# fperezgamonal/flownet2-tf

Measured on AMD Instinct MI355X. Metric: forward pairs/sec at 512x384 (FlowNet2), higher is better.
Workload: dtype f16x2 (split fp16 hi+lo operands, 3 fp16 MFMAs per product, fp32 accumulate); 1 GPU; FlowNet2 forward, batch=4 synthetic 512x384 pairs per GPU, seeded synthetic weights; pairs_per_gpu=4, parallelism=dp1 (no collective)

## Files before the change

flownet2-tf_amd/csrc/conv.hip:

```cpp
#include "conv_common.h"
#include <cstdlib>

namespace fn2 {

template <typename T, typename OutT, int TC, int WC, int WP>
__global__ void __launch_bounds__(256) conv_igemm_kernel(const ConvArgs p) {
  constexpr int CH = 16 / (int)sizeof(T);
  constexpr int BC = WC * TC * 16;
  constexpr int BP = WP * 64;
  constexpr int NT = 256;
  static_assert(WC * WP == 4, "4 waves per block");
  constexpr int NPR = BP / 64;
  constexpr int NWR = (BC * 4 + NT - 1) / NT;
  constexpr int WSWZ_BIT = (TC == 4) ? 5 : (TC == 2) ? 4 : 3;
  __shared__ uint4 lds[2][(BC + BP) * 4];

  const int tid = threadIdx.x, lane = tid & 63, wave = tid >> 6;
  const int wc = wave / WP, wp = wave % WP;
  const int cid = tid & 3;

  int pad_y = p.pad, pad_x = p.pad, oy_off = 0, ox_off = 0, osc = 1;
  const T* wgt = reinterpret_cast<const T*>(p.wgt);
  const int phase = blockIdx.z / p.splitk, split = blockIdx.z - phase * p.splitk;
  if (p.deconv) {
// ... 167 lines not shown
               p.out_c0;
#pragma unroll
    for (int t = 0; t < TC; ++t) {
      float v[4];
      const int co = cout_base + t * 4;
#pragma unroll
      for (int r = 0; r < 4; ++r) {
        float x = acc[t][pt][r] * p.out_scale + bias[t][r];
        if constexpr (sizeof(OutT) == 4) {
          if (p.accum && co + r < p.Cout) x += load_elem<OutT>(po + co + r);
          if (co + r < p.Cout) x = act_grad<OutT>(p, out, po + co + r, co + r, x);
        }
        if (p.act == FN2_ACT_LEAKY) x = leaky(x);
        v[r] = x;
      }
      if (p.vec_ok && co + 3 < p.Cout) {
        store4<OutT>(po + co, v[0], v[1], v[2], v[3]);
      } else {
#pragma unroll
        for (int r = 0; r < 4; ++r)
          if (co + r < p.Cout) store_elem<OutT>(po + co + r, v[r]);
      }
    }
  }
}

template <typename OutT>
__global__ void __launch_bounds__(256) splitk_finalize_kernel(const float* __restrict__ ws, const float* __restrict__ bias,
                                                              OutT* __restrict__ out, long npix, int ws_cs, int splitk,
                                                              int Cout, int out_cs, int out_c0, int act, int vec_ok,
                                                              float out_scale, int accum, const OutT* __restrict__ mask_y,
                                                              int mask_c0, int mask_c1, const float* __restrict__ up_src,
                                                              const float* __restrict__ up_w, const float* __restrict__ up_bias,
                                                              int up_c0, int out_H, int out_W) {
  const int groups = ws_cs / 4;
  const int groups_all = groups + (up_src != nullptr ? 1 : 0);
  const long total = npix * groups_all;
  const size_t slab = (size_t)npix * ws_cs;
  for (long i = (long)blockIdx.x * blockDim.x + threadIdx.x; i < total; i += (long)gridDim.x * blockDim.x) {
    const long pix = i / groups_all;
    const int co = (int)(i - pix * groups_all) * 4;
    if (co == groups * 4) {
      const int ox = (int)(pix % out_W), oy = (int)((pix / out_W) % out_H), n = (int)(pix / out_W / out_H);
      const int H = out_H >> 1, W = out_W >> 1;
      const int a = oy & 1, b = ox & 1, y = oy >> 1, x = ox >> 1;
      float r0 = up_bias ? up_bias[0] : 0.f, r1 = up_bias ? up_bias[1] : 0.f;
#pragma unroll
      for (int ty = 0; ty < 2; ++ty) {
        const int iy = y - 1 + a + ty, ky = 3 - a - 2 * ty;
        if (iy < 0 || iy >= H) continue;
#pragma unroll
        for (int tx = 0; tx < 2; ++tx) {
          const int ix = x - 1 + b + tx, kx = 3 - b - 2 * tx;
          if (ix < 0 || ix >= W) continue;
          const float2 v = *reinterpret_cast<const float2*>(up_src + (((long)n * H + iy) * W + ix) * 2);
          const float* ww = up_w + (ky * 4 + kx) * 4;
          r0 += v.x * ww[0] + v.y * ww[1];
          r1 += v.x * ww[2] + v.y * ww[3];
        }
      }
      OutT* pu = out + (size_t)pix * out_cs + up_c0;
      store_elem<OutT>(pu, r0);
      store_elem<OutT>(pu + 1, r1);
      continue;
    }
    float4 v = *reinterpret_cast<const float4*>(ws + pix * ws_cs + co);
    int s = 1;
    for (; s + 3 < splitk; s += 4) {
      float4 t[4];
#pragma unroll
      for (int u = 0; u < 4; ++u) t[u] = *reinterpret_cast<const float4*>(ws + (s + u) * slab + pix * ws_cs + co);
#pragma unroll
      for (int u = 0; u < 4; ++u) { v.x += t[u].x; v.y += t[u].y; v.z += t[u].z; v.w += t[u].w; }
    }
    for (; s < splitk; ++s) {
      const float4 t = *reinterpret_cast<const float4*>(ws + s * slab + pix * ws_cs + co);
      v.x += t.x; v.y += t.y; v.z += t.z; v.w += t.w;
    }
    float r[4] = {v.x, v.y, v.z, v.w};
    OutT* po = out + (size_t)pix * out_cs + out_c0 + co;
    const bool full = vec_ok && co + 3 < Cout;
    float old[4] = {0.f, 0.f, 0.f, 0.f}, yv[4] = {1.f, 1.f, 1.f, 1.f};
    const bool mask = mask_y != nullptr && co < mask_c1 && co + 4 > mask_c0;
    if constexpr (sizeof(OutT) == 4) {
      if (full) {
        if (accum) load4<OutT>(po, old);
        if (mask) load4<OutT>(mask_y + (size_t)pix * out_cs + out_c0 + co, yv);
      } else {
#pragma unroll
        for (int j = 0; j < 4; ++j)
          if (co + j < Cout) {
            if (accum) old[j] = load_elem<OutT>(po + j);
            if (mask) yv[j] = load_elem<OutT>(mask_y + (size_t)pix * out_cs + out_c0 + co + j);
          }
      }
    }
#pragma unroll
    for (int j = 0; j < 4; ++j) {
      r[j] *= out_scale;
      if (bias != nullptr && co + j < Cout) r[j] += bias[co + j];
// ... 697 lines not shown
  if (d->wgt_layout >= 1) {
    const long in_bytes = (long)d->in.n * d->in.h * d->in.w * d->in.cs * esz;
    FN2_REQUIRE(in_bytes < (1L << 31), "conv2d: input buffer >= 2 GiB is not addressable by the LDS-DMA kernel");
    FN2_REQUIRE((long)d->cout_pad * d->kpad * esz < (1L << 31), "conv2d: packed weight >= 2 GiB per phase");
    a.in_bytes = (int)in_bytes;
  }
  {
    const double A = (double)d->cout_pad * d->kpad * esz, B = (double)d->in.n * d->in.h * d->in.w * d->in.cs * esz;
    const long X = cdiv(M, 64), Y = cdiv(d->cout_pad, 128);
    const char* e = getenv("FN2_WMAJOR");
    const int mode = e ? atoi(e) : 2;
    a.wmajor = mode == 2 ? (A * (double)(X < 8 ? X : 8) + B > A + B * (double)(Y < 8 ? Y : 8)) : mode;
  }
  a.bp64 = wfrag ? 1 : wants_bp64(a, tile, phases, d->wgt_layout) ? 1 : 0;
  if ((a.dbg & 64) && d->wgt_layout == 1 && tile == 128 && !a.bp64) a.bp64 = 2;
  if (wfrag) {
    const char* e_wr = getenv("FN2_WREG_RING");
    const char* e_ring = getenv("FN2_RING_MAX");
    const int mode = e_wr ? atoi(e_wr) : 1;
    const long blocks = (long)cdiv(a.M, 64) * (a.cout_pad / 128) * phases;
    if (tile == 128 && (mode == 2 || (mode == 1 && blocks >= 384 && blocks <= (e_ring ? atoi(e_ring) : 512)))) a.wfrag = 2;
  }
  a.kg = 1;
  if (d->wgt_layout == 1 && tile == 128 && !(a.dbg & 32)) {
    const char* e_kg = getenv("FN2_KG");
    if (!e_kg || atoi(e_kg) != 0) {
      const char* e3 = getenv("FN2_KG3_MAX");
      const char* e2 = getenv("FN2_KG2_MAX");
      const long blocks = (long)cdiv(a.M, 64) * (a.cout_pad / 128) * phases;
      if (blocks <= (e3 ? atoi(e3) : 0)) { a.bp64 = 1; a.kg = 3; }
      else if (blocks <= (e2 ? atoi(e2) : 95)) { a.bp64 = 1; a.kg = 2; }
    }
  }
  if (d->wgt_layout == 1 && tile == 128 && !(a.dbg & 32) && d->in.dtype == FN2_F16X2) {
    const char* e_lo = getenv("FN2_DEEP_MIN");
    const char* e_hi = getenv("FN2_DEEP_MAX");
    const long blocks = (long)cdiv(a.M, 64) * (a.cout_pad / 128) * phases;
    const int lo = e_lo ? atoi(e_lo) : 0, hi = e_hi ? atoi(e_hi) : -1;
    if (blocks >= lo && blocks <= hi) { a.bp64 = 3; a.kg = 1; }
  }
  if (d->wgt_layout == 1 && tile == 128 && a.bp64 == 1 && a.kg == 1) {
    const char* e_ring = getenv("FN2_RING_MAX");
    const int ring_max = e_ring ? atoi(e_ring) : 512;
    const long blocks = (long)cdiv(a.M, 64) * (a.cout_pad / 128) * phases;
    if ((a.dbg & 256) || (blocks >= 384 && blocks <= ring_max)) a.bp64 = 2;
    const char* e_rs = getenv("FN2_RING_SPLIT");
    if (e_rs && blocks >= atoi(e_rs) && blocks < 384) a.bp64 = 2;
  }
  *tile_out = tile;
  *phases_out = phases;
  return FN2_OK;
}

static int preferred_split(const ConvArgs& a, int tile, int phases) {
  if (a.merged) return 1;
  const int bp = tile == 128 ? (a.bp64 ? 64 : 128) : (a.bp64 ? 128 : 256);
  const long blocks = (long)cdiv(a.M, bp) * (a.cout_pad / tile) * phases;
  const char* e_min = getenv("FN2_SPLIT_MINBLOCKS");
  if (blocks >= (e_min ? atoi(e_min) : 384)) return 1;
  if (a.bp64 == 3) {
    const char* e_sl = getenv("FN2_DEEP_SLOTS");
    int s = (int)((e_sl ? atoi(e_sl) : 256) / blocks);
    const int maxs = a.ksteps / 16;
    if (s > maxs) s = maxs;
    if (s > 16) s = 16;
    if (s < 2) return 1;
    const int kper = cdiv(a.ksteps, s);
    return cdiv(a.ksteps, kper);
  }
  if (a.kg > 1) {
    const char* e_nos = getenv("FN2_KG_NOSPLIT");
    if (blocks >= (e_nos ? atoi(e_nos) : 96)) return 1;
    const char* e_sl = getenv("FN2_KG_SLOTS");
    int s = (int)((e_sl ? atoi(e_sl) : 256) / blocks);
    const int maxs = a.ksteps / (12 * a.kg);
    if (s > maxs) s = maxs;
    if (s > 16) s = 16;
    if (s < 2) return 1;
    const int kper = cdiv(a.ksteps, s);
    return cdiv(a.ksteps, kper);
  }
  const char* e = getenv("FN2_SPLIT_SLOTS");
  const char* e_rsl = getenv("FN2_RING_SPLIT_SLOTS");
  const int slots = (tile == 128 && a.bp64 == 2) ? (e_rsl ? atoi(e_rsl) : 512) : e ? atoi(e) : 640;
  int s = (int)(slots / blocks);
  const int maxs = a.ksteps / 8;
  if (s > maxs) s = maxs;
  if (s > 16) s = 16;
  if (s < 2) return 1;
  const int kper = cdiv(a.ksteps, s);
  return cdiv(a.ksteps, kper);
}

static int64_t split_bytes(const ConvArgs& a, int s) {
  return (int64_t)s * a.N * a.out_H * a.out_W * a.ws_cs * (int64_t)sizeof(float);
}

}

extern "C" {

int64_t fn2_conv2d_workspace_bytes(const fn2_conv_desc* d) {
  ConvArgs a;
  int tile, phases;
  if (build_args(d, &a, &tile, &phases) != FN2_OK) return 0;
  if (is_flow_head(d)) return 0;
  const int s = preferred_split(a, tile, phases);
  return s > 1 ? split_bytes(a, s) : 0;
}

int fn2_conv2d_splits(const fn2_conv_desc* d) {
  ConvArgs a;
  int tile, phases;
  if (build_args(d, &a, &tile, &phases) != FN2_OK || is_flow_head(d)) return 1;
  int sk = preferred_split(a, tile, phases);
  while (sk > 1 && (d->workspace == nullptr || split_bytes(a, sk) > d->workspace_bytes)) --sk;
  if ((long)a.N * a.out_H * a.out_W * a.ws_cs >= (1L << 31)) sk = 1;
  if (sk > 1) {
    const int kper = cdiv(a.ksteps, sk);
    sk = cdiv(a.ksteps, kper);
    if (d->wgt_layout >= 1) sk = cdiv(a.ksteps / 2, cdiv(kper, 2));
  }
  return sk < 1 ? 1 : sk;
}

int fn2_conv2d_kernel_name(const fn2_conv_desc* d, char* name, int cap) {
  FN2_REQUIRE(name && cap > 0, "conv2d_kernel_name: no buffer");
  name[0] = 0;
  if (!d || d->wgt_layout < 1 || is_flow_head(d)) return FN2_OK;
  conv_name_sink() = ConvNameSink{name, cap};
  const int rc = fn2_conv2d(d, nullptr);
  conv_name_sink() = ConvNameSink{nullptr, 0};
  return rc;
}

int fn2_conv2d(const fn2_conv_desc* d, void* stream) {
  ConvArgs a;
  int tile, phases;
  int rc = build_args(d, &a, &tile, &phases);
  if (rc) return rc;
  hipStream_t s = (hipStream_t)stream;
  if (is_flow_head(d)) {
    int blocks = grid_for((long)a.M * 64, 256);
    if (d->in.dtype == FN2_F16X2 && a.M <= 4096 && !(a.dbg & 32768)) {
      a.dbg |= 16384;
      blocks = a.M;
    } else {
      a.dbg &= ~16384;
    }
    if (d->in.dtype == FN2_F32)
      hipLaunchKernelGGL(flow_head_kernel<float>, dim3(blocks), dim3(256), 0, s, a);
    else if (d->in.dtype == FN2_BF16)
      hipLaunchKernelGGL(flow_head_kernel<bf16_t>, dim3(blocks), dim3(256), 0, s, a);
    else if (d->in.dtype == FN2_F16)
      hipLaunchKernelGGL(flow_head_kernel<f16_t>, dim3(blocks), dim3(256), 0, s, a);
    else
      hipLaunchKernelGGL(flow_head_kernel<x2_t>, dim3(blocks), dim3(256), 0, s, a);
    FN2_CHECK_LAUNCH("flow_head");
    return FN2_OK;
  }
  int sk = preferred_split(a, tile, phases);
  while (sk > 1 && (d->workspace == nullptr || split_bytes(a, sk) > d->workspace_bytes)) --sk;
  if ((long)a.N * a.out_H * a.out_W * a.ws_cs >= (1L << 31)) sk = 1;
  if (sk > 1) {
    a.kper = cdiv(a.ksteps, sk);
    sk = cdiv(a.ksteps, a.kper);
  }
  if (sk > 1) {
    a.splitk = sk;
    a.ws = reinterpret_cast<float*>(d->workspace);
  }
  if (d->up_src != nullptr && d->kind == 5 && 2 * d->out.c == 32) {
    a.up_src = d->up_src; a.up_w = d->up_w; a.up_bias = d->up_bias; a.up_c0 = d->up_c0;
  }
  if (d->head != nullptr && !conv_name_sink().buf) {
    const fn2_conv_desc* h = reinterpret_cast<const fn2_conv_desc*>(d->head);
    FN2_REQUIRE(d->kind == 1 && is_flow_head(h) && h->head == nullptr && h->up_src == nullptr,
                "conv2d: head rides on a kind-1 transposed conv and is a 3x3 two-output fp32 flow head");
    FN2_REQUIRE(h->in.data == d->in.data && h->in.n == d->in.n && h->in.h == d->in.h && h->in.w == d->in.w &&
                    h->in.cs == d->in.cs && h->in.c0 == d->in.c0 && h->in.dtype == d->in.dtype,
                "conv2d: head and transposed conv must read the same view");
    ConvArgs ha;
    int htile, hphases;
    rc = build_args(h, &ha, &htile, &hphases);
    if (rc) return rc;
    const char* e = getenv("FN2_HEAD_RIDE");
    const bool ride = d->in.dtype == FN2_F16X2 && d->wgt_layout == 2 && tile == 128 && sk > 1 && !(e && atoi(e) == 0);
    if (ride) {
      a.fh_M = ha.M;
      a.fh_w = reinterpret_cast<const float*>(ha.wgt);
      a.fh_w1 = ha.ksteps * 4 * 4;
      a.fh_groups = ha.cin_chunks >> 1;
      a.fh_bias = ha.bias;
      a.fh_out = reinterpret_cast<float*>(ha.out);
      a.fh_out_cs = ha.out_cs; a.fh_out_c0 = ha.out_c0;
      a.fh_scale = ha.out_scale;
    } else {
      rc = fn2_conv2d(h, stream);
      if (rc) return rc;
    }
  }
  if (d->wgt_layout >= 1) {
    a.ksteps = a.ksteps / 2;
    a.kper = cdiv(a.kper, 2);
    a.splitk = cdiv(a.ksteps, a.kper);
    if (a.splitk == 1) a.ws = nullptr;
    rc = launch_conv_fast(a, d->in.dtype, d->out.dtype, tile, phases, s);
  } else if (d->in.dtype == FN2_F32 && d->out.dtype == FN2_F16X2) rc = launch_conv<float, x2_t>(a, tile, phases, s);
  else if (d->in.dtype == FN2_F32) rc = launch_conv<float, float>(a, tile, phases, s);
  else if (d->in.dtype == FN2_BF16 && d->out.dtype == FN2_BF16) rc = launch_conv<bf16_t, bf16_t>(a, tile, phases, s);
  else if (d->in.dtype == FN2_BF16) rc = launch_conv<bf16_t, float>(a, tile, phases, s);
  else if (d->out.dtype == FN2_F16) rc = launch_conv<f16_t, f16_t>(a, tile, phases, s);
  else rc = launch_conv<f16_t, float>(a, tile, phases, s);
  if (rc || conv_name_sink().buf) return rc;
  if (a.splitk == 1) {
    if (d->up_src == nullptr || a.up_src != nullptr) return rc;
    fn2_tensor uv = d->out;
    uv.c = 2; uv.c0 = d->up_c0;
    return fn2_upsample_flow(d->up_src, d->up_w, d->up_bias, &uv, d->out.n, d->out.h / 2, d->out.w / 2, stream);
  }
  if ((a.dbg & 524288) || d->raw_partials) return rc;
  const long npix = (long)a.N * a.out_H * a.out_W;
  const int fgrid = grid_for(npix * (a.ws_cs / 4 + (d->up_src != nullptr ? 1 : 0)), 256);
  if (d->out.dtype == FN2_F32)
    hipLaunchKernelGGL(splitk_finalize_kernel<float>, dim3(fgrid), dim3(256), 0, s, a.ws, a.bias, (float*)a.out, npix,
                       a.ws_cs, a.splitk, a.Cout, a.out_cs, a.out_c0, a.act, a.vec_ok, a.out_scale, a.accum, (const float*)a.mask_y, a.mask_c0, a.mask_c1, d->up_src, d->up_w, d->up_bias, d->up_c0, a.out_H, a.out_W);
  else if (d->out.dtype == FN2_F16X2)
    hipLaunchKernelGGL(splitk_finalize_kernel<x2_t>, dim3(fgrid), dim3(256), 0, s, a.ws, a.bias, (x2_t*)a.out,
                       npix, a.ws_cs, a.splitk, a.Cout, a.out_cs, a.out_c0, a.act, a.vec_ok, a.out_scale, a.accum, (const x2_t*)a.mask_y, a.mask_c0, a.mask_c1, d->up_src, d->up_w, d->up_bias, d->up_c0, a.out_H, a.out_W);
  else if (d->out.dtype == FN2_BF16)
    hipLaunchKernelGGL(splitk_finalize_kernel<bf16_t>, dim3(fgrid), dim3(256), 0, s, a.ws, a.bias, (bf16_t*)a.out,
                       npix, a.ws_cs, a.splitk, a.Cout, a.out_cs, a.out_c0, a.act, a.vec_ok, a.out_scale, a.accum, (const bf16_t*)a.mask_y, a.mask_c0, a.mask_c1, d->up_src, d->up_w, d->up_bias, d->up_c0, a.out_H, a.out_W);
  else
    hipLaunchKernelGGL(splitk_finalize_kernel<f16_t>, dim3(fgrid), dim3(256), 0, s, a.ws, a.bias, (f16_t*)a.out,
                       npix, a.ws_cs, a.splitk, a.Cout, a.out_cs, a.out_c0, a.act, a.vec_ok, a.out_scale, a.accum, (const f16_t*)a.mask_y, a.mask_c0, a.mask_c1, d->up_src, d->up_w, d->up_bias, d->up_c0, a.out_H, a.out_W);
  FN2_CHECK_LAUNCH("splitk_finalize");
  return FN2_OK;
}

int fn2_flow_head_gather(const float* t, int t_cs, const float* bias, float* out, int n, int h, int w, void* stream) {
  FN2_REQUIRE(t && out, "flow_head_gather: null pointer");
  FN2_REQUIRE(t_cs >= 18 && t_cs % 2 == 0 && n >= 1 && h >= 1 && w >= 1, "flow_head_gather: t must hold 18 partials per pixel");
  const long tiles = (long)n * ((h + GT_Y - 1) / GT_Y) * ((w + GT_X - 1) / GT_X);
  if (tiles >= 1024)
    hipLaunchKernelGGL(flow_head_gather_kernel, dim3((unsigned)std::min<long>(tiles, 1 << 16)), dim3(256), 0,
                       (hipStream_t)stream, t, t_cs, bias, out, n, h, w);
  else
    hipLaunchKernelGGL(flow_head_gather_small_kernel, dim3(grid_for((long)n * h * w, 256)), dim3(256), 0,
                       (hipStream_t)stream, t, t_cs, bias, out, n, h, w);
  FN2_CHECK_LAUNCH("flow_head_gather");
  return FN2_OK;
}

int fn2_flow_head_tail(const float* t, int t_cs, int taps, const float* bias, float* pf, int n, int h, int w, int ring,
                       const float* up_w, const float* up_bias, const fn2_tensor* up_out, void* stream) {
  return fn2_flow_head_tail_slabs(t, t_cs, 1, 0, 1.f, taps, bias, pf, n, h, w, ring, up_w, up_bias, up_out, stream);
}

int fn2_flow_head_tail_slabs(const float* t, int t_cs, int nslab, int64_t slab_stride, float scale, int taps, const float* bias,
                             float* pf, int n, int h, int w, int ring, const float* up_w, const float* up_bias,
                             const fn2_tensor* up_out, void* stream) {
  FN2_REQUIRE(t && pf, "flow_head_tail: null pointer");
  FN2_REQUIRE(nslab >= 1 && (nslab == 1 || slab_stride >= (int64_t)n * h * w * t_cs), "flow_head_tail: bad slab geometry");
  const TailSrc ts{t, t_cs, nslab, (long)slab_stride, scale};
  FN2_REQUIRE(taps == 3 || taps == 5, "flow_head_tail: taps must be 3 or 5");
  FN2_REQUIRE(t_cs >= 2 * taps * taps && t_cs % 2 == 0 && n >= 1 && h >= 1 && w >= 1,
              "flow_head_tail: t must hold 2 * taps^2 partials per pixel");
  FN2_REQUIRE(!ring || (h >= 3 && w >= 3), "flow_head_tail: a border ring needs h, w >= 3");
// ... 154 lines not shown
```

flownet2-tf_amd/csrc/conv2.hip:

```cpp
#include "conv_common.h"

#include <type_traits>
#include <algorithm>
#include <utility>

#ifndef FN2_X2_ORDER
#define FN2_X2_ORDER 0
#endif
#ifndef FN2_CONV_ABLATE
#define FN2_CONV_ABLATE 0
#endif
#ifndef FN2_SETPRIO
#define FN2_SETPRIO 1
#endif

namespace fn2 {

typedef __attribute__((address_space(3))) void* lptr_t;

constexpr unsigned kOobOffset = 0x80000000u;

typedef int v4i_t __attribute__((ext_vector_type(4)));
typedef unsigned u32x4_t __attribute__((ext_vector_type(4)));

// ... 64 lines not shown
    a0 += __shfl_xor(a0, off, 64);
    a1 += __shfl_xor(a1, off, 64);
  }
  if (lane == 0)
    *reinterpret_cast<float2*>(pf + (((size_t)n * H + y) * W + x) * 2) = make_float2(a0 + p.h5_bc[2 * cs], a1 + p.h5_bc[2 * cs + 1]);
}

__device__ __forceinline__ void h5_ring_block(const ConvArgs& p, int rb) {
  const int wave = threadIdx.x >> 6;
  const long total = (long)p.N * (2 * p.OW + 2 * (p.OH - 2));
  for (int k = 0; k < 4; ++k) {
    const long m = (long)rb * 16 + wave * 4 + k;
    if (m >= total) return;
    h5_ring_pixel(p, m);
  }
}

__device__ __forceinline__ float* h5_t(uint4* a, uint4* b, int half, int w) {
  const int byte = w * 4;
  return byte < half ? reinterpret_cast<float*>(reinterpret_cast<char*>(a) + byte)
                     : reinterpret_cast<float*>(reinterpret_cast<char*>(b) + (byte - half));
}

template <typename T, typename OutT, int WC, int WP, int TCN = 2, int TPN = 2, int STAGES = 2, int KG = 1, bool M16 = false,
          bool WREG = false, bool SLAB = false, bool HEAD5 = false, bool FEED = false>
__global__ void __launch_bounds__(256 * KG + (FEED ? 256 : 0)) conv_igemm2_kernel(const ConvArgs p) {
#if defined(__HIP_DEVICE_COMPILE__)
  constexpr int CH = 16 / (int)sizeof(T);
  constexpr int ESZ = (int)sizeof(T);
  constexpr int BC = WC * TCN * 32, BP = WP * TPN * 32;
  static_assert(WC * WP == 4, "4 waves per block");
  constexpr int NWI = BC / 32;
  constexpr int NPI = BP / 32;
  static_assert(!WREG || (is_x2<T>::value && TCN == 1 && KG == 1 && (STAGES == 2 || STAGES == 3) && !M16),
                "WREG: split fp16, one cout tile per wave, two-stage loop or 3-slot ring");
  constexpr int BOFF = WREG ? 0 : BC;
  constexpr int kWTileBytes = (32 * TPN * (TCN * 32 + 4) + 32 * TPN) * 4;
  constexpr int kPoolHalfRows = (STAGES * BP * 128 / 2 > 2 * kWTileBytes ? STAGES * BP * 128 / 2 : 2 * kWTileBytes) / 128 + 1;
  constexpr int ROWS = WREG ? kPoolHalfRows : BC + BP;
  static_assert(KG == 1 || STAGES == 2, "K groups run the two-stage loop");
  constexpr bool kDeep = STAGES > 3;
  __shared__ uint4 lds0_all[(kDeep ? STAGES : WREG ? 2 : KG) * ROWS * 8];
  __shared__ uint4 lds1_all[(kDeep || WREG) ? 1 : KG * ROWS * 8];
  __shared__ uint4 lds2_own[(STAGES == 3 && !WREG) ? ROWS * 8 : 1];

  if constexpr (HEAD5) {
    if ((int)blockIdx.x >= p.h5_tiles) {
      h5_ring_block(p, (int)blockIdx.x - p.h5_tiles);
      return;
    }
  }
  if constexpr (WREG && SLAB && is_x2<T>::value) {
    if (p.fh_M > 0 && (int)blockIdx.z >= p.fh_z0) {
      if (FEED && threadIdx.x >= 256) return;
      float* part = reinterpret_cast<float*>(lds0_all);
      const long e = (((long)blockIdx.z - p.fh_z0) * gridDim.y + blockIdx.y) * gridDim.x + blockIdx.x;
      const long total = (long)(gridDim.z - p.fh_z0) * gridDim.y * gridDim.x;
      for (long m = e; m < p.fh_M; m += total)
        fh_pixel(reinterpret_cast<const x2_t*>(p.in), p.H, p.W, p.in_cs, p.in_c0, p.fh_groups, p.fh_w, p.fh_w + p.fh_w1,
                 p.fh_bias, p.fh_scale, p.fh_out + (size_t)m * p.fh_out_cs + p.fh_out_c0, m, part);
      return;
    }
  }
  const int tid = threadIdx.x, lane = tid & 63;
  const int wave_all = __builtin_amdgcn_readfirstlane(tid >> 6);
  const int grp = KG > 1 ? wave_all >> 2 : 0;
  static_assert(!FEED || (WREG && STAGES == 3 && KG == 1), "FEED: the WREG ring");
  const bool feeder = FEED && wave_all >= 4;
  const int wave = (KG > 1 || FEED) ? wave_all & 3 : wave_all;
  uint4* const lds0 = lds0_all + grp * (ROWS * 8);
  uint4* const lds1 = WREG ? lds0_all + BP * 8 : kDeep ? lds0_all + ROWS * 8 : lds1_all + grp * (ROWS * 8);
  uint4* const lds2 = WREG ? lds0_all + 2 * BP * 8 : lds2_own;
  uint4* const ep1 = (kDeep || WREG) ? lds0_all + ROWS * 8 : lds1_all;
  const int wc = wave / WP, wp = wave % WP;

  int pad_y = p.pad, pad_x = p.pad, oy_off = 0, ox_off = 0, osc = 1;
  const T* wgt = reinterpret_cast<const T*>(p.wgt);
  const int phase = blockIdx.z / p.splitk, split = blockIdx.z - phase * p.splitk;
  const unsigned wrow_bytes = (unsigned)p.ksteps * 128u;
  if (p.deconv) {
    const int a = phase >> 1, b = phase & 1;
    pad_y = a ? p.ph_pad1 : p.ph_pad0; pad_x = b ? p.ph_pad1 : p.ph_pad0; oy_off = a; ox_off = b; osc = 2;
    wgt += (size_t)phase * p.cout_pad * (wrow_bytes / ESZ);
  }
  const int khi = p.deconv ? p.kh_ph[phase >> 1] : p.KH, kwi = p.deconv ? p.kw_ph[phase & 1] : p.KW;
  const int nst_all = (p.cin_chunks >> 3) * khi * kwi;
  const int kt0 = split * p.kper + grp;
  const int kt1 = (FN2_CONV_ABLATE && (p.dbg & 1048576)) ? kt0 : min(nst_all, split * p.kper + p.kper);
  int bx = blockIdx.x, by = blockIdx.y;
  if (!(p.dbg & 4)) {
    const int NT = HEAD5 ? p.h5_tiles : gridDim.x * gridDim.y, L = blockIdx.x + gridDim.x * blockIdx.y;
    const int xcd = L & 7, chunk = NT >> 3, rem = NT & 7;
    const int Lp = xcd * chunk + min(xcd, rem) + (L >> 3);
    if (p.wmajor) {
      by = Lp / (int)gridDim.x;
      bx = Lp - by * (int)gridDim.x;
    } else {
      bx = Lp / (int)gridDim.y;
      by = Lp - bx * (int)gridDim.y;
    }
  }
  const int m0 = bx * BP;
  const int c0 = by * BC;

// ... 263 lines not shown
      auto w_stage = [&](u32x4_t (&wf)[4]) { load_w(wf); advance(); };
      auto sync_c = [&](u32x4_t (&wf)[4]) {
        asm volatile("s_waitcnt vmcnt(4)\n\ts_barrier" : "+v"(wf[0]), "+v"(wf[1]), "+v"(wf[2]), "+v"(wf[3]) :: "memory");
      };
      w_stage(wfa);
      w_stage(wfb);
      for (int s = 0; s < nst3; s += 3) {
        sync_c(wfa); w_stage(wfc); compute_w(lds0, wfa);
        sync_c(wfb); w_stage(wfa); compute_w(lds1, wfb);
        sync_c(wfc); w_stage(wfb); compute_w(lds2, wfc);
      }
      asm volatile("s_waitcnt vmcnt(0)" : "+v"(wfa[0]), "+v"(wfa[1]), "+v"(wfa[2]), "+v"(wfa[3]), "+v"(wfb[0]), "+v"(wfb[1]),
                   "+v"(wfb[2]), "+v"(wfb[3]) :: "memory");
    }
  } else if constexpr (WREG && STAGES == 3) {
    static_assert(NPI + 4 == 6, "vmcnt literal below");
    auto ring_sync_w = [&](u32x4_t (&wf)[4]) {
      asm volatile("s_waitcnt vmcnt(6)\n\ts_barrier" : "+v"(wf[0]), "+v"(wf[1]), "+v"(wf[2]), "+v"(wf[3]) :: "memory");
    };
    issue_stage_w(lds0, wfa);
    issue_stage_w(lds1, wfb);
    const int nst3 = (kt1 - kt0 + 2) / 3 * 3;
    for (int s = 0; s < nst3; s += 3) {
      ring_sync_w(wfa); issue_stage_w(lds2, wfc); compute_w(lds0, wfa);
      ring_sync_w(wfb); issue_stage_w(lds0, wfa); compute_w(lds1, wfb);
      ring_sync_w(wfc); issue_stage_w(lds1, wfb); compute_w(lds2, wfc);
    }
    asm volatile("s_waitcnt vmcnt(0)" : "+v"(wfa[0]), "+v"(wfa[1]), "+v"(wfa[2]), "+v"(wfa[3]), "+v"(wfb[0]), "+v"(wfb[1]),
                 "+v"(wfb[2]), "+v"(wfb[3]) :: "memory");
  } else if constexpr (WREG) {
    issue_stage_w(lds0, wfa);
    wait_w(wfa);
    __syncthreads();
    const int nst2 = (kt1 - kt0 + 1) & ~1;
    for (int s = 0; s < nst2; s += 2) {
      issue_stage_w(lds1, wfb);
      compute_w(lds0, wfa);
      wait_w(wfb);
      __syncthreads();
      if (s + 2 < nst2) issue_stage_w(lds0, wfa);
      compute_w(lds1, wfb);
      wait_w(wfa);
      __syncthreads();
    }
  } else if constexpr (STAGES == 2) {
    issue_stage(lds0);
    asm volatile("s_waitcnt vmcnt(0)" ::: "memory");
    __syncthreads();
    const int nst2 = ((kt1 - (kt0 - grp) + KG - 1) / KG + 1) & ~1;
    for (int s = 0; s < nst2; s += 2) {
      issue_stage(lds1);
      compute(lds0);
      asm volatile("s_waitcnt vmcnt(0)" ::: "memory");
      __syncthreads();
      if (s + 2 < nst2) issue_stage(lds0);
      compute(lds1);
      asm volatile("s_waitcnt vmcnt(0)" ::: "memory");
      __syncthreads();
    }
  } else if constexpr (kDeep) {
    constexpr int ND = NWI + NPI, D = STAGES - 1;
    static_assert(ND * (D - 1) <= 63, "vmcnt field");
    auto slot_ptr = [&](int sl) { return lds0_all + sl * (ROWS * 8); };
#pragma unroll
    for (int d = 0; d < D; ++d) issue_stage(slot_ptr(d));
    const int nst = kt1 - kt0;
    int rd = 0, wr = D;
    for (int s = 0; s < nst; ++s) {
      asm volatile("s_waitcnt vmcnt(%0)\n\ts_barrier" :: "n"(ND * (D - 1)) : "memory");
      issue_stage(slot_ptr(wr));
      compute(slot_ptr(rd));
      rd = rd + 1 == STAGES ? 0 : rd + 1;
      wr = wr + 1 == STAGES ? 0 : wr + 1;
    }
    asm volatile("s_waitcnt vmcnt(0)" ::: "memory");
  } else {
    constexpr int ND = NWI + NPI;
    static_assert(ND == 5 || ND == 6 || ND == 8, "vmcnt literal below");
    auto ring_sync = [] {
      if constexpr (ND == 5) asm volatile("s_waitcnt vmcnt(5)\n\ts_barrier" ::: "memory");
      else if constexpr (ND == 6) asm volatile("s_waitcnt vmcnt(6)\n\ts_barrier" ::: "memory");
      else asm volatile("s_waitcnt vmcnt(8)\n\ts_barrier" ::: "memory");
    };
    issue_stage(lds0);
    issue_stage(lds1);
    const int nst3 = (kt1 - kt0 + 2) / 3 * 3;
    for (int s = 0; s < nst3; s += 3) {
      ring_sync(); issue_stage(lds2); compute(lds0);
      ring_sync(); issue_stage(lds0); compute(lds1);
      ring_sync(); issue_stage(lds1); compute(lds2);
    }
    asm volatile("s_waitcnt vmcnt(0)" ::: "memory");
  }

  if constexpr (KG > 1) {
    constexpr int NA4 = TCN * TPN * 4;
    static_assert((KG - 1) * 4 * NA4 * 64 <= KG * ROWS * 8, "reduction scratch must fit the stage buffers");
    float4* red = reinterpret_cast<float4*>(lds0_all);
    auto acc4 = [&](int idx) -> float4 {
      if constexpr (M16) {
        const f32x4 v = acc16[idx / (TPN * 2)][idx % (TPN * 2)];
        return make_float4(v[0], v[1], v[2], v[3]);
      } else {
        const int t = idx >> 2, q = idx & 3;
        return make_float4(acc[t / TPN][t % TPN][4 * q], acc[t / TPN][t % TPN][4 * q + 1], acc[t / TPN][t % TPN][4 * q + 2],
                           acc[t / TPN][t % TPN][4 * q + 3]);
      }
    };
    if (grp > 0) {
#pragma unroll
      for (int idx = 0; idx < NA4; ++idx) red[(((grp - 1) * 4 + wave) * NA4 + idx) * 64 + lane] = acc4(idx);
    }
    __syncthreads();
    if (grp > 0) return;
#pragma unroll
    for (int g = 0; g < KG - 1; ++g)
#pragma unroll
      for (int idx = 0; idx < NA4; ++idx) {
        const float4 v = red[((g * 4 + wave) * NA4 + idx) * 64 + lane];
        if constexpr (M16) {
          f32x4& d = acc16[idx / (TPN * 2)][idx % (TPN * 2)];
          d[0] += v.x; d[1] += v.y; d[2] += v.z; d[3] += v.w;
        } else {
          const int t = idx >> 2, q = idx & 3;
          acc[t / TPN][t % TPN][4 * q] += v.x; acc[t / TPN][t % TPN][4 * q + 1] += v.y;
          acc[t / TPN][t % TPN][4 * q + 2] += v.z; acc[t / TPN][t % TPN][4 * q + 3] += v.w;
        }
      }
  }

  if constexpr (HEAD5) {
    if (p.dbg & 2) return;
    constexpr int TS = 52;
    static_assert(256 * TS * 4 <= 2 * ROWS * 128, "T fits the stage buffers");
#pragma unroll
    for (int tc = 0; tc < TCN; ++tc)
#pragma unroll
      for (int tp = 0; tp < TPN; ++tp) {
        const int pos = wp * TPN * 32 + tp * 32 + fr;
        const int cb = tc * 32 + fh * 16;
#pragma unroll
        for (int q = 0; q < 4; ++q)
          if (cb + 4 * q < TS)
            *reinterpret_cast<float4*>(h5_t(lds0_all, lds1_all, ROWS * 128, pos * TS + cb + 4 * q)) =
                make_float4(acc[tc][tp][4 * q] * p.out_scale, acc[tc][tp][4 * q + 1] * p.out_scale,
                            acc[tc][tp][4 * q + 2] * p.out_scale, acc[tc][tp][4 * q + 3] * p.out_scale);
      }
    __syncthreads();
    if (p.dbg & 8) return;
    const int tx = bx % p.h5_tx, tyn = bx / p.h5_tx;
    const int n = tyn / p.h5_ty, ty = tyn - n * p.h5_ty;
    float* pf = reinterpret_cast<float*>(p.out);
// ... 30 lines not shown
#pragma unroll
      for (int a = 0; a < TCN * 2; ++a) {
        const int co = c0 + wc * TCN * 32 + (a >> 1) * 32 + 16 * (g16 & 1) + 8 * (a & 1) + 4 * (g16 >> 1);
        if (slab != nullptr) {
          if (co < p.ws_cs)
            *reinterpret_cast<float4*>(slab + opix * p.ws_cs + co) =
                make_float4(acc16[a][b][0], acc16[a][b][1], acc16[a][b][2], acc16[a][b][3]);
          continue;
        }
        float v[4];
#pragma unroll
        for (int j = 0; j < 4; ++j) {
          float x = acc16[a][b][j] * p.out_scale + ((p.bias != nullptr && co + j < p.Cout) ? p.bias[co + j] : 0.f);
          if constexpr (sizeof(OutT) == 4) {
            if (p.accum && co + j < p.Cout) x += load_elem<OutT>(po + co + j);
            if (co + j < p.Cout) x = act_grad<OutT>(p, out16, po + co + j, co + j, x);
          }
          if (p.act == FN2_ACT_LEAKY) x = leaky(x);
          v[j] = x;
        }
        if (p.vec_ok && co + 3 < p.Cout) store_vec<OutT, 4>(po + co, v);
        else
#pragma unroll
          for (int j = 0; j < 4; ++j)
            if (co + j < p.Cout) store_elem<OutT>(po + co + j, v[j]);
      }
    }
    return;
  }

  OutT* out = reinterpret_cast<OutT*>(p.out);
  constexpr int WCOLS = TCN * 32, RS = WCOLS + 4, WROWS = 32 * TPN;
  constexpr int WTW = WROWS * RS + WROWS;
  constexpr bool kLdsT = (KG > 1 ? 4 : 2) * WTW * 4 <= KG * ROWS * 128;
  if constexpr (FEED && !kLdsT) { if (feeder) return; }
  float* const tl = reinterpret_cast<float*>(KG > 1 ? ep1 : (wave < 2 ? lds0_all : ep1)) + (KG > 1 ? wave : (wave & 1)) * WTW;
  constexpr int CPR = WCOLS / 4, RPI = 64 / CPR;
  static_assert(!SLAB || WREG, "SLAB is a specialisation of the WREG instantiations");
  if ((SLAB || !WREG) && p.splitk > 1) {
    float* slab = p.ws + (size_t)split * p.N * p.out_H * p.out_W * p.ws_cs;
    if constexpr (kLdsT) {
      if constexpr (STAGES >= 3) __syncthreads();
      if constexpr (FEED) { if (feeder) return; }
      int* rowoff = reinterpret_cast<int*>(tl + WROWS * RS);
#pragma unroll
      for (int tp = 0; tp < TPN; ++tp) {
        const int m = m0 + wp * TPN * 32 + tp * 32 + fr;
        const int mm = m < p.M ? m : 0;
        const int n = mm / (p.OH * p.OW);
        const int rem = mm - n * (p.OH * p.OW);
        const int oy = rem / p.OW, ox = rem - oy * p.OW;
        if (fh == 0) rowoff[tp * 32 + fr] = m < p.M ? (int)((((size_t)n * p.out_H + (oy * osc + oy_off)) * p.out_W + (ox * osc + ox_off)) * p.ws_cs) : -1;
#pragma unroll
        for (int tc = 0; tc < TCN; ++tc)
#pragma unroll
          for (int q = 0; q < 4; ++q)
            *reinterpret_cast<float4*>(tl + (tp * 32 + fr) * RS + tc * 32 + fh * 16 + q * 4) =
                make_float4(acc[tc][tp][4 * q], acc[tc][tp][4 * q + 1], acc[tc][tp][4 * q + 2], acc[tc][tp][4 * q + 3]);
      }
      const int rr = lane / CPR, ch = lane - rr * CPR;
      const int co = c0 + wc * WCOLS + ch * 4;
#pragma unroll
      for (int i = 0; i < WROWS / RPI; ++i) {
        const int row = i * RPI + rr;
        const float4 v = *reinterpret_cast<const float4*>(tl + row * RS + ch * 4);
        const int off = rowoff[row];
        if (off >= 0 && co < p.ws_cs) *reinterpret_cast<float4*>(slab + (size_t)off + co) = v;
      }
      return;
// ... 799 lines not shown
    if (conv_name_sink().buf)                                                                          \
      snprintf(conv_name_sink().buf, conv_name_sink().cap, "conv_igemm2_kernel<%s, %s, %s, %s>", type_name<T>(), \
               type_name<OutT>(), #__VA_ARGS__, m16 ? "true" : "false");                              \
    else if (m16) hipLaunchKernelGGL((conv_igemm2_kernel<T, OutT, __VA_ARGS__, is_x2<T>::value>), grid, dim3(THREADS), 0, s, a); \
    else hipLaunchKernelGGL((conv_igemm2_kernel<T, OutT, __VA_ARGS__, false>), grid, dim3(THREADS), 0, s, a);            \
  } while (0)
  if (a.wfrag) {
    if constexpr (is_x2<T>::value) {
      if (tile == 64) {
        dim3 grid(cdiv(a.M, 128), a.cout_pad / 64, z);
        if (conv_name_sink().buf)
          snprintf(conv_name_sink().buf, conv_name_sink().cap, "conv_igemm2_kernel<%s, %s, 2, 2, 1, 2, 2, 1, false, true, %s>",
                   type_name<T>(), type_name<OutT>(), a.splitk > 1 ? "true" : "false");
        else if (a.splitk > 1)
          hipLaunchKernelGGL((conv_igemm2_kernel<T, OutT, 2, 2, 1, 2, 2, 1, false, true, true>), grid, dim3(256), 0, s, a);
        else
          hipLaunchKernelGGL((conv_igemm2_kernel<T, OutT, 2, 2, 1, 2, 2, 1, false, true, false>), grid, dim3(256), 0, s, a);
      } else {
        dim3 grid(cdiv(a.M, 64), a.cout_pad / 128, z);
        const bool slab = a.splitk > 1;
        ConvArgs ah = a;
        if (a.fh_M > 0 && slab && !conv_name_sink().buf) {
          const char* e = getenv("FN2_FH_BLOCKS");
          const long per_z = (long)grid.x * grid.y;
          const long want = std::min<long>(a.fh_M, e ? atoi(e) : 1024);
          ah.fh_z0 = z;
          grid.z = z + (unsigned)std::max<long>(1, (want + per_z - 1) / per_z);
        } else {
          ah.fh_M = 0;
        }
        const ConvArgs& a = ah;
        const char* e_feed = getenv("FN2_WREG_FEED");
        const int feed = e_feed ? atoi(e_feed) : 1;
        if (conv_name_sink().buf)
          snprintf(conv_name_sink().buf, conv_name_sink().cap, "conv_igemm2_kernel<%s, %s, 4, 1, 1, 2, %d, 1, false, true, %s%s>",
                   type_name<T>(), type_name<OutT>(), a.wfrag == 2 ? 3 : 2, slab ? "true" : "false",
                   (a.wfrag == 2 && (slab ? feed >= 2 : feed >= 1)) ? ", false, true" : "");
        else if (a.wfrag == 2 && slab && feed >= 2)
          hipLaunchKernelGGL((conv_igemm2_kernel<T, OutT, 4, 1, 1, 2, 3, 1, false, true, true, false, true>), grid, dim3(512), 0, s, a);
        else if (a.wfrag == 2 && slab)
          hipLaunchKernelGGL((conv_igemm2_kernel<T, OutT, 4, 1, 1, 2, 3, 1, false, true, true>), grid, dim3(256), 0, s, a);
        else if (a.wfrag == 2 && feed >= 1)
          hipLaunchKernelGGL((conv_igemm2_kernel<T, OutT, 4, 1, 1, 2, 3, 1, false, true, false, false, true>), grid, dim3(512), 0, s, a);
        else if (a.wfrag == 2)
          hipLaunchKernelGGL((conv_igemm2_kernel<T, OutT, 4, 1, 1, 2, 3, 1, false, true, false>), grid, dim3(256), 0, s, a);
        else if (slab)
          hipLaunchKernelGGL((conv_igemm2_kernel<T, OutT, 4, 1, 1, 2, 2, 1, false, true, true>), grid, dim3(256), 0, s, a);
        else
          hipLaunchKernelGGL((conv_igemm2_kernel<T, OutT, 4, 1, 1, 2, 2, 1, false, true, false>), grid, dim3(256), 0, s, a);
      }
    } else {
      return fail(FN2_ERR_UNSUPPORTED, "conv fast path: fragment-order weights are split fp16 only");
    }
  } else if (tile == 128 && a.bp64 && a.kg == 3) FN2_LAUNCH2(cdiv(a.M, 64), a.cout_pad / 128, 768, 2, 2, 2, 1, 2, 3);
  else if (tile == 128 && a.bp64 && a.kg == 2) FN2_LAUNCH2(cdiv(a.M, 64), a.cout_pad / 128, 512, 2, 2, 2, 1, 2, 2);
  else if (tile == 128 && a.bp64 == 3) FN2_LAUNCH2(cdiv(a.M, 64), a.cout_pad / 128, 256, 2, 2, 2, 1, 6, 1);
  else if (tile == 128 && a.bp64 == 2) FN2_LAUNCH2(cdiv(a.M, 64), a.cout_pad / 128, 256, 2, 2, 2, 1, 3, 1);
  else if (tile == 128 && a.bp64) FN2_LAUNCH2(cdiv(a.M, 64), a.cout_pad / 128, 256, 2, 2, 2, 1, 2, 1);
  else if (tile == 128) FN2_LAUNCH2(cdiv(a.M, 128), a.cout_pad / 128, 256, 2, 2, 2, 2, 2, 1);
  else if (tile == 64 && a.bp64) FN2_LAUNCH2(cdiv(a.M, 128), a.cout_pad / 64, 256, 1, 4, 2, 1, 2, 1);
  else if (tile == 64) FN2_LAUNCH2(cdiv(a.M, 256), a.cout_pad / 64, 256, 1, 4, 2, 2, 2, 1);
  else if (a.bp64) FN2_LAUNCH2(cdiv(a.M, 128), a.cout_pad / 32, 256, 1, 4, 1, 1, 2, 1);
  else FN2_LAUNCH2(cdiv(a.M, 256), a.cout_pad / 32, 256, 1, 4, 1, 2, 2, 1);
#undef FN2_LAUNCH2
  FN2_CHECK_LAUNCH("conv_igemm2");
  return FN2_OK;
}

int launch_head5_strip(const ConvArgs& a, int blocks, hipStream_t s) {
  if (a.ksteps == 3) hipLaunchKernelGGL((head5_strip_kernel<1>), dim3(blocks), dim3(512), 0, s, a);
// ... 43 lines not shown
```

Before: 1110 pairs/s.

## Add two K-group split path for register-weight conv and wide split-K finalize

Enables two in-block K groups (512 threads) for the fragment-order register-weight conv kernel on small-grid layers. The groups reduce their partial sums through the LDS pool, which is resized and re-strided to hold the extra stage buffers and reduction scratch. The split-K slot heuristic is retuned for these layers, and the ksteps halving now runs before the head-ride decision. The finalize kernel gains a seven-wide unrolled load path for split counts of 6 to 8, so all partial slabs are loaded before they are summed. This trades higher LDS use and more reduction work for better latency hiding on low-occupancy layers.

```diff
diff --git a/flownet2-tf_amd/csrc/conv.hip b/flownet2-tf_amd/csrc/conv.hip
--- a/flownet2-tf_amd/csrc/conv.hip
+++ b/flownet2-tf_amd/csrc/conv.hip
@@ -223,7 +223,7 @@
                                                               float out_scale, int accum, const OutT* __restrict__ mask_y,
                                                               int mask_c0, int mask_c1, const float* __restrict__ up_src,
                                                               const float* __restrict__ up_w, const float* __restrict__ up_bias,
-                                                              int up_c0, int out_H, int out_W) {
+                                                              int up_c0, int out_H, int out_W, int wide) {
   const int groups = ws_cs / 4;
   const int groups_all = groups + (up_src != nullptr ? 1 : 0);
   const long total = npix * groups_all;
@@ -257,6 +257,15 @@
     }
     float4 v = *reinterpret_cast<const float4*>(ws + pix * ws_cs + co);
     int s = 1;
+    if (wide) {
+      float4 t[7];
+#pragma unroll
+      for (int u = 0; u < 7; ++u) t[u] = *reinterpret_cast<const float4*>(ws + min(1 + u, splitk - 1) * slab + pix * ws_cs + co);
+#pragma unroll
+      for (int u = 0; u < 7; ++u)
+        if (1 + u < splitk) { v.x += t[u].x; v.y += t[u].y; v.z += t[u].z; v.w += t[u].w; }
+      s = splitk;
+    }
     for (; s + 3 < splitk; s += 4) {
       float4 t[4];
 #pragma unroll
@@ -1020,6 +1029,14 @@
       else if (blocks <= (e2 ? atoi(e2) : 95)) { a.bp64 = 1; a.kg = 2; }
     }
   }
+  if (wfrag && a.wfrag == 1 && tile == 128 && !(a.dbg & 32)) {
+    const char* e_kg = getenv("FN2_KG");
+    if (!e_kg || atoi(e_kg) != 0) {
+      const char* e2 = getenv("FN2_KG2_MAX");
+      const long blocks = (long)cdiv(a.M, 64) * (a.cout_pad / 128) * phases;
+      if (blocks <= (e2 ? atoi(e2) : 95)) a.kg = 2;
+    }
+  }
   if (d->wgt_layout == 1 && tile == 128 && !(a.dbg & 32) && d->in.dtype == FN2_F16X2) {
     const char* e_lo = getenv("FN2_DEEP_MIN");
     const char* e_hi = getenv("FN2_DEEP_MAX");
@@ -1061,6 +1078,13 @@
     if (blocks >= (e_nos ? atoi(e_nos) : 96)) return 1;
     const char* e_sl = getenv("FN2_KG_SLOTS");
     int s = (int)((e_sl ? atoi(e_sl) : 256) / blocks);
+    if (a.wfrag && !e_sl) {
+      const char* e = getenv("FN2_SPLIT_SLOTS");
+      int plain = (int)((e ? atoi(e) : 640) / blocks);
+      if (plain > a.ksteps / 8) plain = a.ksteps / 8;
+      if (plain > 16) plain = 16;
+      s = cdiv(plain, a.kg);
+    }
     const int maxs = a.ksteps / (12 * a.kg);
     if (s > maxs) s = maxs;
     if (s > 16) s = 16;
@@ -1080,6 +1104,15 @@
   return cdiv(a.ksteps, kper);
 }
 
+static int preferred_split_groups(ConvArgs& a, int tile, int phases) {
+  int s = preferred_split(a, tile, phases);
+  if (a.wfrag && a.kg > 1 && s < 2) {
+    a.kg = 1;
+    s = preferred_split(a, tile, phases);
+  }
+  return s;
+}
+
 static int64_t split_bytes(const ConvArgs& a, int s) {
   return (int64_t)s * a.N * a.out_H * a.out_W * a.ws_cs * (int64_t)sizeof(float);
 }
@@ -1093,7 +1126,7 @@
   int tile, phases;
   if (build_args(d, &a, &tile, &phases) != FN2_OK) return 0;
   if (is_flow_head(d)) return 0;
-  const int s = preferred_split(a, tile, phases);
+  const int s = preferred_split_groups(a, tile, phases);
   return s > 1 ? split_bytes(a, s) : 0;
 }
 
@@ -1101,7 +1134,7 @@
   ConvArgs a;
   int tile, phases;
   if (build_args(d, &a, &tile, &phases) != FN2_OK || is_flow_head(d)) return 1;
-  int sk = preferred_split(a, tile, phases);
+  int sk = preferred_split_groups(a, tile, phases);
   while (sk > 1 && (d->workspace == nullptr || split_bytes(a, sk) > d->workspace_bytes)) --sk;
   if ((long)a.N * a.out_H * a.out_W * a.ws_cs >= (1L << 31)) sk = 1;
   if (sk > 1) {
@@ -1147,7 +1180,7 @@
     FN2_CHECK_LAUNCH("flow_head");
     return FN2_OK;
   }
-  int sk = preferred_split(a, tile, phases);
+  int sk = preferred_split_groups(a, tile, phases);
   while (sk > 1 && (d->workspace == nullptr || split_bytes(a, sk) > d->workspace_bytes)) --sk;
   if ((long)a.N * a.out_H * a.out_W * a.ws_cs >= (1L << 31)) sk = 1;
   if (sk > 1) {
@@ -1158,6 +1191,13 @@
     a.splitk = sk;
     a.ws = reinterpret_cast<float*>(d->workspace);
   }
+  if (d->wgt_layout >= 1) {
+    a.ksteps = a.ksteps / 2;
+    a.kper = cdiv(a.kper, 2);
+    a.splitk = cdiv(a.ksteps, a.kper);
+    if (a.splitk == 1) a.ws = nullptr;
+  }
+  if (a.splitk == 1) a.kg = a.wfrag ? 1 : a.kg;
   if (d->up_src != nullptr && d->kind == 5 && 2 * d->out.c == 32) {
     a.up_src = d->up_src; a.up_w = d->up_w; a.up_bias = d->up_bias; a.up_c0 = d->up_c0;
   }
@@ -1173,7 +1213,7 @@
     rc = build_args(h, &ha, &htile, &hphases);
     if (rc) return rc;
     const char* e = getenv("FN2_HEAD_RIDE");
-    const bool ride = d->in.dtype == FN2_F16X2 && d->wgt_layout == 2 && tile == 128 && sk > 1 && !(e && atoi(e) == 0);
+    const bool ride = d->in.dtype == FN2_F16X2 && d->wgt_layout == 2 && tile == 128 && a.splitk > 1 && !(e && atoi(e) == 0);
     if (ride) {
       a.fh_M = ha.M;
       a.fh_w = reinterpret_cast<const float*>(ha.wgt);
@@ -1188,11 +1228,8 @@
       if (rc) return rc;
     }
   }
+  FN2_REQUIRE(a.fh_M == 0 || a.splitk > 1, "conv2d: a riding head needs the K-split launch");
   if (d->wgt_layout >= 1) {
-    a.ksteps = a.ksteps / 2;
-    a.kper = cdiv(a.kper, 2);
-    a.splitk = cdiv(a.ksteps, a.kper);
-    if (a.splitk == 1) a.ws = nullptr;
     rc = launch_conv_fast(a, d->in.dtype, d->out.dtype, tile, phases, s);
   } else if (d->in.dtype == FN2_F32 && d->out.dtype == FN2_F16X2) rc = launch_conv<float, x2_t>(a, tile, phases, s);
   else if (d->in.dtype == FN2_F32) rc = launch_conv<float, float>(a, tile, phases, s);
@@ -1210,18 +1247,19 @@
   if ((a.dbg & 524288) || d->raw_partials) return rc;
   const long npix = (long)a.N * a.out_H * a.out_W;
   const int fgrid = grid_for(npix * (a.ws_cs / 4 + (d->up_src != nullptr ? 1 : 0)), 256);
+  const int wide = a.splitk > 5 && a.splitk <= 8 && !(a.dbg & 8388608);
   if (d->out.dtype == FN2_F32)
     hipLaunchKernelGGL(splitk_finalize_kernel<float>, dim3(fgrid), dim3(256), 0, s, a.ws, a.bias, (float*)a.out, npix,
-                       a.ws_cs, a.splitk, a.Cout, a.out_cs, a.out_c0, a.act, a.vec_ok, a.out_scale, a.accum, (const float*)a.mask_y, a.mask_c0, a.mask_c1, d->up_src, d->up_w, d->up_bias, d->up_c0, a.out_H, a.out_W);
+                       a.ws_cs, a.splitk, a.Cout, a.out_cs, a.out_c0, a.act, a.vec_ok, a.out_scale, a.accum, (const float*)a.mask_y, a.mask_c0, a.mask_c1, d->up_src, d->up_w, d->up_bias, d->up_c0, a.out_H, a.out_W, wide);
   else if (d->out.dtype == FN2_F16X2)
     hipLaunchKernelGGL(splitk_finalize_kernel<x2_t>, dim3(fgrid), dim3(256), 0, s, a.ws, a.bias, (x2_t*)a.out,
-                       npix, a.ws_cs, a.splitk, a.Cout, a.out_cs, a.out_c0, a.act, a.vec_ok, a.out_scale, a.accum, (const x2_t*)a.mask_y, a.mask_c0, a.mask_c1, d->up_src, d->up_w, d->up_bias, d->up_c0, a.out_H, a.out_W);
+                       npix, a.ws_cs, a.splitk, a.Cout, a.out_cs, a.out_c0, a.act, a.vec_ok, a.out_scale, a.accum, (const x2_t*)a.mask_y, a.mask_c0, a.mask_c1, d->up_src, d->up_w, d->up_bias, d->up_c0, a.out_H, a.out_W, wide);
   else if (d->out.dtype == FN2_BF16)
     hipLaunchKernelGGL(splitk_finalize_kernel<bf16_t>, dim3(fgrid), dim3(256), 0, s, a.ws, a.bias, (bf16_t*)a.out,
-                       npix, a.ws_cs, a.splitk, a.Cout, a.out_cs, a.out_c0, a.act, a.vec_ok, a.out_scale, a.accum, (const bf16_t*)a.mask_y, a.mask_c0, a.mask_c1, d->up_src, d->up_w, d->up_bias, d->up_c0, a.out_H, a.out_W);
+                       npix, a.ws_cs, a.splitk, a.Cout, a.out_cs, a.out_c0, a.act, a.vec_ok, a.out_scale, a.accum, (const bf16_t*)a.mask_y, a.mask_c0, a.mask_c1, d->up_src, d->up_w, d->up_bias, d->up_c0, a.out_H, a.out_W, wide);
   else
     hipLaunchKernelGGL(splitk_finalize_kernel<f16_t>, dim3(fgrid), dim3(256), 0, s, a.ws, a.bias, (f16_t*)a.out,
-                       npix, a.ws_cs, a.splitk, a.Cout, a.out_cs, a.out_c0, a.act, a.vec_ok, a.out_scale, a.accum, (const f16_t*)a.mask_y, a.mask_c0, a.mask_c1, d->up_src, d->up_w, d->up_bias, d->up_c0, a.out_H, a.out_W);
+                       npix, a.ws_cs, a.splitk, a.Cout, a.out_cs, a.out_c0, a.act, a.vec_ok, a.out_scale, a.accum, (const f16_t*)a.mask_y, a.mask_c0, a.mask_c1, d->up_src, d->up_w, d->up_bias, d->up_c0, a.out_H, a.out_W, wide);
   FN2_CHECK_LAUNCH("splitk_finalize");
   return FN2_OK;
 }
diff --git a/flownet2-tf_amd/csrc/conv2.hip b/flownet2-tf_amd/csrc/conv2.hip
--- a/flownet2-tf_amd/csrc/conv2.hip
+++ b/flownet2-tf_amd/csrc/conv2.hip
@@ -120,11 +120,13 @@
   static_assert(WC * WP == 4, "4 waves per block");
   constexpr int NWI = BC / 32;
   constexpr int NPI = BP / 32;
-  static_assert(!WREG || (is_x2<T>::value && TCN == 1 && KG == 1 && (STAGES == 2 || STAGES == 3) && !M16),
+  static_assert(!WREG || (is_x2<T>::value && TCN == 1 && (STAGES == 2 || STAGES == 3) && !M16),
                 "WREG: split fp16, one cout tile per wave, two-stage loop or 3-slot ring");
+  static_assert(!WREG || KG == 1 || (SLAB && STAGES == 2 && !FEED), "WREG K groups: the K-split two-stage loop only");
   constexpr int BOFF = WREG ? 0 : BC;
   constexpr int kWTileBytes = (32 * TPN * (TCN * 32 + 4) + 32 * TPN) * 4;
-  constexpr int kPoolHalfRows = (STAGES * BP * 128 / 2 > 2 * kWTileBytes ? STAGES * BP * 128 / 2 : 2 * kWTileBytes) / 128 + 1;
+  constexpr int kPoolStageHalf = KG * STAGES * BP * 128 / 2, kPoolTileHalf = (KG > 2 ? KG - 1 : 1) * 2 * kWTileBytes;
+  constexpr int kPoolHalfRows = (kPoolStageHalf > kPoolTileHalf ? kPoolStageHalf : kPoolTileHalf) / 128 + 1;
   constexpr int ROWS = WREG ? kPoolHalfRows : BC + BP;
   static_assert(KG == 1 || STAGES == 2, "K groups run the two-stage loop");
   constexpr bool kDeep = STAGES > 3;
@@ -140,7 +142,7 @@
   }
   if constexpr (WREG && SLAB && is_x2<T>::value) {
     if (p.fh_M > 0 && (int)blockIdx.z >= p.fh_z0) {
-      if (FEED && threadIdx.x >= 256) return;
+      if ((FEED || KG > 1) && threadIdx.x >= 256) return;
       float* part = reinterpret_cast<float*>(lds0_all);
       const long e = (((long)blockIdx.z - p.fh_z0) * gridDim.y + blockIdx.y) * gridDim.x + blockIdx.x;
       const long total = (long)(gridDim.z - p.fh_z0) * gridDim.y * gridDim.x;
@@ -156,8 +158,8 @@
   static_assert(!FEED || (WREG && STAGES == 3 && KG == 1), "FEED: the WREG ring");
   const bool feeder = FEED && wave_all >= 4;
   const int wave = (KG > 1 || FEED) ? wave_all & 3 : wave_all;
-  uint4* const lds0 = lds0_all + grp * (ROWS * 8);
-  uint4* const lds1 = WREG ? lds0_all + BP * 8 : kDeep ? lds0_all + ROWS * 8 : lds1_all + grp * (ROWS * 8);
+  uint4* const lds0 = lds0_all + grp * (WREG ? 2 * BP * 8 : ROWS * 8);
+  uint4* const lds1 = WREG ? lds0 + BP * 8 : kDeep ? lds0_all + ROWS * 8 : lds1_all + grp * (ROWS * 8);
   uint4* const lds2 = WREG ? lds0_all + 2 * BP * 8 : lds2_own;
   uint4* const ep1 = (kDeep || WREG) ? lds0_all + ROWS * 8 : lds1_all;
   const int wc = wave / WP, wp = wave % WP;
@@ -487,7 +489,7 @@
     issue_stage_w(lds0, wfa);
     wait_w(wfa);
     __syncthreads();
-    const int nst2 = (kt1 - kt0 + 1) & ~1;
+    const int nst2 = ((kt1 - (kt0 - grp) + KG - 1) / KG + 1) & ~1;
     for (int s = 0; s < nst2; s += 2) {
       issue_stage_w(lds1, wfb);
       compute_w(lds0, wfa);
@@ -550,7 +552,9 @@
 
   if constexpr (KG > 1) {
     constexpr int NA4 = TCN * TPN * 4;
-    static_assert((KG - 1) * 4 * NA4 * 64 <= KG * ROWS * 8, "reduction scratch must fit the stage buffers");
+    constexpr int kRedStride = WREG ? kWTileBytes / 16 : NA4 * 64;
+    static_assert(NA4 * 64 <= kRedStride && kWTileBytes % 16 == 0, "a wave's accumulators fit its region");
+    static_assert((KG - 1) * 4 * kRedStride <= (WREG ? 2 : KG) * ROWS * 8, "reduction scratch must fit the stage buffers");
     float4* red = reinterpret_cast<float4*>(lds0_all);
     auto acc4 = [&](int idx) -> float4 {
       if constexpr (M16) {
@@ -564,7 +568,7 @@
     };
     if (grp > 0) {
 #pragma unroll
-      for (int idx = 0; idx < NA4; ++idx) red[(((grp - 1) * 4 + wave) * NA4 + idx) * 64 + lane] = acc4(idx);
+      for (int idx = 0; idx < NA4; ++idx) red[((grp - 1) * 4 + wave) * kRedStride + idx * 64 + lane] = acc4(idx);
     }
     __syncthreads();
     if (grp > 0) return;
@@ -572,7 +576,7 @@
     for (int g = 0; g < KG - 1; ++g)
 #pragma unroll
       for (int idx = 0; idx < NA4; ++idx) {
-        const float4 v = red[((g * 4 + wave) * NA4 + idx) * 64 + lane];
+        const float4 v = red[(g * 4 + wave) * kRedStride + idx * 64 + lane];
         if constexpr (M16) {
           f32x4& d = acc16[idx / (TPN * 2)][idx % (TPN * 2)];
           d[0] += v.x; d[1] += v.y; d[2] += v.z; d[3] += v.w;
@@ -669,9 +673,11 @@
   OutT* out = reinterpret_cast<OutT*>(p.out);
   constexpr int WCOLS = TCN * 32, RS = WCOLS + 4, WROWS = 32 * TPN;
   constexpr int WTW = WROWS * RS + WROWS;
-  constexpr bool kLdsT = (KG > 1 ? 4 : 2) * WTW * 4 <= KG * ROWS * 128;
+  static_assert(!WREG || WTW * 4 == kWTileBytes, "the pool is sized for these tiles");
+  constexpr bool kLdsT = (WREG && KG > 1) ? 4 * WTW * 4 <= 2 * ROWS * 128 : (KG > 1 ? 4 : 2) * WTW * 4 <= KG * ROWS * 128;
   if constexpr (FEED && !kLdsT) { if (feeder) return; }
-  float* const tl = reinterpret_cast<float*>(KG > 1 ? ep1 : (wave < 2 ? lds0_all : ep1)) + (KG > 1 ? wave : (wave & 1)) * WTW;
+  float* const tl = (WREG && KG > 1) ? reinterpret_cast<float*>(lds0_all) + wave * WTW
+                                     : reinterpret_cast<float*>(KG > 1 ? ep1 : (wave < 2 ? lds0_all : ep1)) + (KG > 1 ? wave : (wave & 1)) * WTW;
   constexpr int CPR = WCOLS / 4, RPI = 64 / CPR;
   static_assert(!SLAB || WREG, "SLAB is a specialisation of the WREG instantiations");
   if ((SLAB || !WREG) && p.splitk > 1) {
@@ -1537,10 +1543,14 @@
         const ConvArgs& a = ah;
         const char* e_feed = getenv("FN2_WREG_FEED");
         const int feed = e_feed ? atoi(e_feed) : 1;
+        const bool kg2 = a.wfrag == 1 && slab && a.kg == 2;
+        if (a.kg != 1 && !kg2) return fail(FN2_ERR_UNSUPPORTED, "conv fast path: %d K groups on this fragment-order launch", a.kg);
         if (conv_name_sink().buf)
-          snprintf(conv_name_sink().buf, conv_name_sink().cap, "conv_igemm2_kernel<%s, %s, 4, 1, 1, 2, %d, 1, false, true, %s%s>",
-                   type_name<T>(), type_name<OutT>(), a.wfrag == 2 ? 3 : 2, slab ? "true" : "false",
+          snprintf(conv_name_sink().buf, conv_name_sink().cap, "conv_igemm2_kernel<%s, %s, 4, 1, 1, 2, %d, %d, false, true, %s%s>",
+                   type_name<T>(), type_name<OutT>(), a.wfrag == 2 ? 3 : 2, kg2 ? 2 : 1, slab ? "true" : "false",
                    (a.wfrag == 2 && (slab ? feed >= 2 : feed >= 1)) ? ", false, true" : "");
+        else if (kg2)
+          hipLaunchKernelGGL((conv_igemm2_kernel<T, OutT, 4, 1, 1, 2, 2, 2, false, true, true>), grid, dim3(512), 0, s, a);
         else if (a.wfrag == 2 && slab && feed >= 2)
           hipLaunchKernelGGL((conv_igemm2_kernel<T, OutT, 4, 1, 1, 2, 3, 1, false, true, true, false, true>), grid, dim3(512), 0, s, a);
         else if (a.wfrag == 2 && slab)
```

New measurement: 1109 pairs/s. No clear change (-0.1%).
